# rpacheco-blazquez/PINN-FEM

Measured on AMD Instinct MI355X. Metric: element-residual-grad evals/sec (PINN+GD iteration: MLP fwd+bwd, stiffness, assembly, residual, Adam), collinear truss, higher is better.
Workload: dtype f32; 1 GPU; ex4 shape (nets (20, 15, 10), E and A evaluated), 1000000 elements per GPU, collinear 2-D truss h=1, alpha_data=100 with measurements at every node, load factor 0.1; elements_total=1000000, parallelism=elements sharded x1

## Files before the change

include/pinnfem_hip.h:

```cpp
#ifndef PINNFEM_HIP_H
#define PINNFEM_HIP_H

#include <stdint.h>

#ifdef __cplusplus
extern "C" {
#endif

#define PF_ABI_VERSION 9

#define PF_OK 0
#define PF_ERR_ARG (-1)
#define PF_ERR_UNSUPPORTED (-2)
#define PF_ERR_HIP (-3)

#define PF_DOF_FIXED 1u
#define PF_DOF_MEASURED 2u
#define PF_DOF_SHARED 4u
#define PF_DOF_GHOST 8u

#define PF_WG_SHUFFLE 0
#define PF_WG_MFMA 1
#define PF_WG_MFMA44 2
#define PF_WG_MFMA32 3
// ... 108 lines not shown
int pf_padded_width(int width);
int pf_net_pad_count(int in_dim, int width, int n_hidden);
int pf_net_pad_index(int in_dim, int width, int n_hidden, int local);
int pf_sizeof(int what);
int pf_net_op_count(int in_dim, int width, int n_hidden);
long long pf_partials_count(const pf_problem* p);
#define PF_FUSED_FORWARD 1
#define PF_FUSED_BACKWARD 2
#define PF_FUSED_THETA_UPDATE 4
#define PF_FUSED_U_PINGPONG 8
#define PF_FUSED_U_UPDATE 16
int pf_fusion_info(const pf_problem* p);
#define PF_GRAPH_FORM_FOLDED_RESIDUAL 1
int pf_graph_form_info(const pf_problem* p);
int pf_graph_light_forward(const pf_problem* p);

int pf_pack_theta(const pf_problem* p, void* stream);
int pf_net_forward(const pf_problem* p, int which, void* stream);
int pf_net_forward_all(const pf_problem* p, void* stream);
int pf_net_backward_all(const pf_problem* p, void* stream);
int pf_internal_force(const pf_problem* p, const float* u, float* f_int_out, void* stream);
int pf_node_residual(const pf_problem* p, float* f_int_out, void* stream);
int pf_elem_adjoint(const pf_problem* p, void* stream);
int pf_net_backward(const pf_problem* p, int which, void* stream);
int pf_node_gradu(const pf_problem* p, int fuse_adam, void* stream);
int pf_theta_reduce(const pf_problem* p, int fuse_adam, void* stream);
int pf_finalize(const pf_problem* p, void* stream);
int pf_reset(const pf_problem* p, void* stream);

int pf_gd_iterations(const pf_problem* p, int n_iter, void* stream);
// ... 177 lines not shown
```

pinn_fem_amd/_capi.py:

```python
from __future__ import annotations

import ctypes as C
import os

_HERE = os.path.dirname(os.path.abspath(__file__))
LIB_PATH = os.environ.get("PINNFEM_LIB") or os.path.join(_HERE, "lib", "libpinnfem_hip.so")

PF_ABI_VERSION = 9
PF_OK, PF_ERR_ARG, PF_ERR_UNSUPPORTED, PF_ERR_HIP = 0, -1, -2, -3
PF_DOF_FIXED, PF_DOF_MEASURED, PF_DOF_SHARED, PF_DOF_GHOST = 1, 2, 4, 8
PF_WG_SHUFFLE, PF_WG_MFMA, PF_WG_MFMA44, PF_WG_MFMA32 = 0, 1, 2, 3
PF_N32_WIDTH_MAX = 30
PF_MLP_F32, PF_MLP_BF16 = 0, 1
PF_FE_REFERENCE, PF_FE_DELTA = 0, 1
PF_HIST_COLS = 6
PF_MAX_BLOCKS = 1024
PF_COMM_ID_BYTES = 128
PF_MAX_NODE_BLOCKS = 4096
PF_NODE_SLOTS = PF_MAX_NODE_BLOCKS + 8
PF_KERNEL_SLOTS = 9
PF_COARSE_MAX_AGG, PF_COARSE_MODES = 256, 3
PF_COARSE_MAX = PF_COARSE_MAX_AGG * PF_COARSE_MODES
PF_PCG_MAX_RHS = 2
PF_DYN_ENERGY_COUNT = 4 + 4 * PF_MAX_NODE_BLOCKS
# ... 102 lines not shown
_PD = C.POINTER(PfDyn)
_PH = C.POINTER(PfDynHist)
SYMBOLS = {
    "pf_abi_version": (C.c_int, []),
    "pf_last_error": (C.c_char_p, []),
    "pf_net_param_count": (C.c_int, [C.c_int, C.c_int, C.c_int]),
    "pf_padded_width": (C.c_int, [C.c_int]),
    "pf_net_pad_count": (C.c_int, [C.c_int, C.c_int, C.c_int]),
    "pf_net_pad_index": (C.c_int, [C.c_int, C.c_int, C.c_int, C.c_int]),
    "pf_sizeof": (C.c_int, [C.c_int]),
    "pf_net_op_count": (C.c_int, [C.c_int, C.c_int, C.c_int]),
    "pf_partials_count": (C.c_longlong, [_PP]),
    "pf_fusion_info": (C.c_int, [_PP]),
    "pf_graph_form_info": (C.c_int, [_PP]),
    "pf_graph_light_forward": (C.c_int, [_PP]),
    "pf_pack_theta": (C.c_int, [_PP, C.c_void_p]),
    "pf_net_forward": (C.c_int, [_PP, C.c_int, C.c_void_p]),
    "pf_net_forward_all": (C.c_int, [_PP, C.c_void_p]),
    "pf_net_backward_all": (C.c_int, [_PP, C.c_void_p]),
    "pf_internal_force": (C.c_int, [_PP, C.c_void_p, C.c_void_p, C.c_void_p]),
    "pf_node_residual": (C.c_int, [_PP, C.c_void_p, C.c_void_p]),
    "pf_elem_adjoint": (C.c_int, [_PP, C.c_void_p]),
    "pf_net_backward": (C.c_int, [_PP, C.c_int, C.c_void_p]),
    "pf_node_gradu": (C.c_int, [_PP, C.c_int, C.c_void_p]),
    "pf_theta_reduce": (C.c_int, [_PP, C.c_int, C.c_void_p]),
    "pf_finalize": (C.c_int, [_PP, C.c_void_p]),
    "pf_reset": (C.c_int, [_PP, C.c_void_p]),
    "pf_gd_iterations": (C.c_int, [_PP, C.c_int, C.c_void_p]),
    "pf_graph_create": (C.c_int, [_PP, C.c_int, C.c_void_p, C.POINTER(C.c_void_p)]),
    "pf_graph_create_ex": (C.c_int, [_PP, C.c_int, C.c_int, C.c_void_p, C.POINTER(C.c_void_p)]),
# ... 141 lines not shown
```

pinn_fem_amd/csrc/pf_api.hip:

```cpp
#include <stdlib.h>
#include <string.h>
#include <stdio.h>
#include "pf_common.h"
#include "pf_graph.h"
#include "pf_net32.h"

int pf_launch_node_residual(const pf_problem* p, float* f_int_out, int compute_loss, hipStream_t s, int fin_prev = 0);
int pf_launch_elem_adjoint(const pf_problem* p, hipStream_t s);
int pf_launch_node_gradu(const pf_problem* p, int fuse_adam, hipStream_t s, int skip_shared = 0, float* u_out = nullptr);
int pf_launch_u_home(const pf_problem* p, hipStream_t s);
int pf_launch_scalar_residual(const pf_problem* p, const pf_scalar_id* sp, hipStream_t s);
int pf_launch_scalar_update(const pf_problem* p, const pf_scalar_id* sp, hipStream_t s);
int pf_launch_shard_pack(const pf_problem* p, float* buf2, const float* u2_local, hipStream_t s);
int pf_launch_shard_update(const pf_problem* p, const float* buf2, float* u2_local, hipStream_t s);
int pf_launch_shard_flush(const pf_problem* p, const float* u2, hipStream_t s);
int pf_launch_theta_reduce(const pf_problem* p, int fuse_adam, hipStream_t s);
int pf_launch_pack_theta(const pf_problem* p, hipStream_t s);
int pf_launch_finalize(const pf_problem* p, int mode, int with_theta, hipStream_t s, int tn_ready = 0);
int pf_launch_theta_stage1(const pf_problem* p, hipStream_t s);
int pf_launch_theta_stage1_path(const pf_problem* p, hipStream_t s, int fin_prev);
int pf_launch_path_check(const pf_problem* p, int* bad, hipStream_t s);
int pf_launch_theta_stage2(const pf_problem* p, int fuse_adam, hipStream_t s);
int pf_launch_reset(const pf_problem* p, hipStream_t s);
int pf_launch_adam(float* param, const float* grad, float* m, float* v, int n, int step, double lr,
// ... 440 lines not shown
}

#define PF_CAP_EV 2

static bool pad_index_is_canonical(const pf_problem* p) {
  const int n = p->n_theta_active;
  if (n <= 0 || !p->pad_index) return false;
  int* h = new int[n];
  const bool ok = hipMemcpy(h, p->pad_index, (size_t)n * sizeof(int), hipMemcpyDeviceToHost) == hipSuccess;
  bool same = ok;
  for (int q = 0; same && q < n; ++q) same = h[q] == pf_pad_index_of(*p, q);
  delete[] h;
  return same;
}

static bool mesh_is_path(const pf_problem* p) {
  const pf_mesh& M = p->mesh;
  if (M.n_elems < 1 || M.n_nodes != M.n_elems + 1 || !M.conn || !M.adj_ptr || !M.adj || !M.dof_flags) return false;
  int* bad = nullptr;
  if (hipMalloc(&bad, sizeof(int)) != hipSuccess) {
    pf_set_error("path check of the mesh failed (hipMalloc): the iteration graph keeps its residual launch");
    return false;
  }
  int h = 1;
  bool ok = hipMemset(bad, 0, sizeof(int)) == hipSuccess && pf_launch_path_check(p, bad, nullptr) == PF_OK &&
            hipMemcpy(&h, bad, sizeof(int), hipMemcpyDeviceToHost) == hipSuccess;
  (void)hipFree(bad);
  if (!ok) pf_set_error("path check of the mesh failed (HIP error): the iteration graph keeps its residual launch");
  return ok && h == 0;
}

static bool can_fold_residual_static(const pf_problem* p) {
  return p->prop_double != 0 && p->elem_k != nullptr && p->u_alt != nullptr && can_fuse_gradu(p) && can_fuse_backward(p) &&
         can_fuse_theta_update(p) && pf_n32_bwd2_has_path(p) && p->n_iface == 0 && p->mesh.dim == p->net[0].in_dim - 1;
}
static bool can_fold_residual(const pf_problem* p) { return can_fold_residual_static(p) && mesh_is_path(p); }
static bool can_light_forward(const pf_problem* p, bool fold) {
  return fold && p->net[0].enabled && p->net[1].enabled && pf_n32_has_light_forward(p);
}

static pf_problem graph_iteration_view(const pf_problem& p, int i) {
  pf_problem q = p;
  if (p.prop_double != 0 && (i & 1)) {
    q.prop_e += q.mesh.n_elems;
    q.prop_a += q.mesh.n_elems;
    if (q.elem_k) q.elem_k += (size_t)q.mesh.n_elems * (q.mesh.dim == 2 ? 3 : 1);
  }
  q.part_half = i & 1;
  return q;
}

static int enqueue_graph_iterations(const pf_problem* p, int iters, const pf_capture& c, bool calc_index = false,
                                    bool head_cont = false, bool no_tail = false, bool fold = false) {
  hipStream_t s = c.s;
  if (!(p->net[0].enabled || p->net[1].enabled)) {
    for (int i = 0; i < iters; ++i) {
      int rc = enqueue_iteration(p, 1, 0, s, nullptr);
      if (rc != PF_OK) return rc;
    }
    return PF_OK;
  }
  const bool fuse_gu = p->prop_double != 0 && p->elem_k != nullptr && can_fuse_gradu(p);
  const bool dag = !fuse_gu && p->mesh.n_elems >= PF_GRAPH_DAG_MIN_ELEMS;
  const bool upp = dag && p->u_alt != nullptr && (iters % 2) == 0;
  const bool fuse_s2 = can_fuse_theta_update(p);
  const int tn_ready = p->wg_mode == PF_WG_MFMA32 ? 1 : 0;
  const size_t k_half = (size_t)p->mesh.n_elems * (p->mesh.dim == 2 ? 3 : 1);
  const bool light = can_light_forward(p, fold);
// ... 1 lines not shown
    hipEvent_t* e = c.ev + PF_CAP_EV * i;
    hipEvent_t* ep = c.ev + PF_CAP_EV * (i - 1);
    pf_problem q = graph_iteration_view(*p, i);
    float* u_next = nullptr;
    if (upp) {
      u_next = (i & 1) ? q.u : q.u_alt;
      if (i & 1) q.u = q.u_alt;
    }
    const bool carries = i > 0 || head_cont;
    pf_fwd2_opts fo;
    if (fuse_s2 && carries) fo.s2_half = (i - 1) & 1;
    fo.calc_index = calc_index;
    if (fuse_gu && carries) {
      fo.gu_nb = pf_node_blocks(q.mesh.n_nodes);
      fo.gu_k = p->elem_k + (((i - 1) & 1) ? k_half : 0);
    }
    if (dag && i > 0 && p->prop_double == 0 && hipStreamWaitEvent(s, ep[1], 0) != hipSuccess)
      return fail(PF_ERR_HIP, "graph edge failed");
    fo.light = light ? 1 : 0;
    PF_TRY(net_forward_all(&q, s, fo), "net_forward");
    if (fold) {
      PF_TRY(net_backward2(&q, s, light ? 2 : 1), "net_backward2");
      PF_TRY(pf_launch_theta_stage1_path(&q, s, carries ? (tn_ready ? 2 : 1) : 0), "theta_stage1");
      if (i == iters - 1 && !no_tail) {
        PF_TRY(pf_launch_theta_stage2(&q, 1, s), "theta_stage2");
        PF_TRY(pf_launch_node_gradu(&q, 1, s, 0, nullptr), "node_gradu");
      }
      continue;
    }
    if (dag && i > 0 && hipStreamWaitEvent(s, ep[1], 0) != hipSuccess) return fail(PF_ERR_HIP, "graph edge failed");
// ... 18 lines not shown
  q.part_half = (iters - 1) & 1;
  PF_TRY(pf_launch_finalize(&q, 0, 0, s, tn_ready), "finalize");
  return PF_OK;
}

int pf_graph_form_info(const pf_problem* p) {
  if (check_problem(p) != PF_OK) return PF_ERR_ARG;
  return can_fold_residual(p) ? PF_GRAPH_FORM_FOLDED_RESIDUAL : 0;
}

int pf_graph_light_forward(const pf_problem* p) {
  if (check_problem(p) != PF_OK) return PF_ERR_ARG;
  return can_light_forward(p, can_fold_residual(p)) ? 1 : 0;
}

int pf_graph_create(const pf_problem* p, int iters_per_graph, void* stream, void** graph_out) {
  return pf_graph_create_ex(p, iters_per_graph, 0, stream, graph_out);
}

static bool can_chain_replays(const pf_problem* p, int iters) {
  return (iters % 2) == 0 && p->prop_double != 0 && p->elem_k != nullptr && can_fuse_gradu(p) && can_fuse_theta_update(p);
}

int pf_graph_create_ex(const pf_problem* p, int iters_per_graph, int flags, void* stream, void** graph_out) {
  int rc = check_gd(p);
  if (rc) return rc;
  if (!graph_out || iters_per_graph < 1) return fail(PF_ERR_ARG, "pf_graph_create_ex: bad argument");
  if ((flags & (PF_GRAPH_CONT_HEAD | PF_GRAPH_NO_TAIL)) && !can_chain_replays(p, iters_per_graph))
    return fail(PF_ERR_UNSUPPORTED, "pf_graph_create_ex: replays of this problem's graph cannot hand over their tail");
  const bool calc_index = can_fuse_theta_update(p) && pad_index_is_canonical(p);
  const bool fold = can_fold_residual(p);
  const bool head = (flags & PF_GRAPH_CONT_HEAD) != 0, no_tail = (flags & PF_GRAPH_NO_TAIL) != 0;
  return capture_graph((hipStream_t)stream, PF_CAP_EV * iters_per_graph, hipStreamCaptureModeThreadLocal, graph_out,
                       [&](pf_capture& cap) { return enqueue_graph_iterations(p, iters_per_graph, cap, calc_index, head, no_tail, fold); });
}

int pf_graph_tail(const pf_problem* p, int iters_per_graph, void* stream) {
  int rc = check_gd(p);
  if (rc) return rc;
  if (!can_chain_replays(p, iters_per_graph)) return fail(PF_ERR_UNSUPPORTED, "pf_graph_tail: not a chained replay");
  hipStream_t s = (hipStream_t)stream;
  const pf_problem q = graph_iteration_view(*p, iters_per_graph - 1);
  PF_TRY(pf_launch_theta_stage2(&q, 1, s), "theta_stage2");
  PF_TRY(pf_launch_node_gradu(&q, 1, s, 0, nullptr), "node_gradu");
  PF_TRY(pf_launch_finalize(&q, 0, 0, s, q.wg_mode == PF_WG_MFMA32 ? 1 : 0), "finalize");
  return PF_OK;
}

int pf_graph_launch(void* graph, void* stream) {
// ... 219 lines not shown
```

pinn_fem_amd/csrc/pf_common.h:

```cpp
#pragma once
#include <hip/hip_runtime.h>
#include <stdint.h>
#include <stdlib.h>
#include "pinnfem_hip.h"

#define PF_WAVE 64

#define PF_PART_R2H(h) ((h) ? 3 * PF_NODE_SLOTS : 0)
#define PF_PART_D2H(h) ((h) ? 4 * PF_NODE_SLOTS : PF_NODE_SLOTS)
#define PF_PART_U2 (2 * PF_NODE_SLOTS)
#define PF_PART_WG (5 * PF_NODE_SLOTS)
#define PF_RG 16

#define PF_NET_THREADS 128
#define PF_NODE_THREADS 256

__host__ __device__ constexpr int pf_pad_w1(int) { return 0; }
__host__ __device__ constexpr int pf_pad_wh(int hp, int l ) {
  return hp * 4 + (l - 2) * hp * (hp + 4);
}
__host__ __device__ constexpr int pf_pad_wo(int hp, int nh) {
  return hp * 4 + (nh - 1) * hp * (hp + 4);
}
__host__ __device__ constexpr int pf_pad_count(int hp, int nh) {
// ... 302 lines not shown
PF_DECL_NET_LAUNCHERS(4)
PF_DECL_NET_LAUNCHERS(8)
PF_DECL_NET_LAUNCHERS(12)
PF_DECL_NET_LAUNCHERS(16)
PF_DECL_NET_LAUNCHERS(20)
PF_DECL_NET_LAUNCHERS(24)
PF_DECL_NET_LAUNCHERS(28)
PF_DECL_NET_LAUNCHERS(32)

struct pf_fwd2_opts {
  int s2_half = -1;
  bool calc_index = false;
  int gu_nb = 0;
  const float* gu_k = nullptr;
  int light = 0;
};
#define PF_DECL_NET32_LAUNCHERS(NRB)                                                       \
  int pf_launch_net32_forward_##NRB(const pf_problem* p, int which, hipStream_t s, int s2_half); \
  int pf_launch_net32_backward_##NRB(const pf_problem* p, int which, hipStream_t s);      \
  int pf_launch_net32_backward_gea_##NRB(const pf_problem* p, int which, hipStream_t s);  \
  int pf_launch_net32b_forward_##NRB(const pf_problem* p, int which, hipStream_t s, int s2_half); \
  int pf_launch_net32b_backward_##NRB(const pf_problem* p, int which, hipStream_t s);     \
  int pf_launch_net32b_backward_gea_##NRB(const pf_problem* p, int which, hipStream_t s); \
  int pf_launch_net32_forward2_##NRB(const pf_problem* p, hipStream_t s, const pf_fwd2_opts& o);    \
  int pf_launch_net32b_forward2_##NRB(const pf_problem* p, hipStream_t s, const pf_fwd2_opts& o);   \
  int pf_launch_net32_backward2_##NRB(const pf_problem* p, hipStream_t s, int path);      \
  int pf_launch_net32b_backward2_##NRB(const pf_problem* p, hipStream_t s, int path);
PF_DECL_NET32_LAUNCHERS(2)
PF_DECL_NET32_LAUNCHERS(4)
PF_DECL_NET32_LAUNCHERS(6)
// ... 15 lines not shown
```

pinn_fem_amd/csrc/pf_mesh.hip:

```cpp
#include <stdlib.h>
#include "pf_common.h"
#include "pf_node.h"
#include "pf_net32.h"


namespace {

template <int DIM>
__device__ __forceinline__ void gather_kv(const pf_problem& P, const float* __restrict__ v, int node,
                                          float* acc, bool own_only = false) {
  const pf_mesh& M = P.mesh;
#pragma unroll
  for (int c = 0; c < DIM; ++c) acc[c] = 0.f;
  const int b = M.adj_ptr[node], e_ = M.adj_ptr[node + 1];
  if (P.adj_other) {
    float vs[2];
    load_vec<DIM>(v, node, vs);
    for (int idx = b; idx < e_; idx += 2) {
      const bool two = idx + 1 < e_;
      const int code0 = M.adj[idx], oth0 = P.adj_other[idx];
      const int code1 = two ? M.adj[idx + 1] : code0, oth1 = two ? P.adj_other[idx + 1] : oth0;
      const int e0 = code0 >> 1, e1 = code1 >> 1;
      const ElemK k0 = load_k<DIM>(P, e0), k1 = load_k<DIM>(P, e1);
      float vo0[2], vo1[2], fe[2];
// ... 250 lines not shown
      if (ok[m]) {
#pragma unroll
        for (int c = 0; c < DIM; ++c) dof_loss_terms(fl[m][c], r[m][c], P.use_data, mv[m][c], un[m][c], sum_r2, sum_d2);
      }
  }
  const float t0 = pf_block_sum(sum_r2, red);
  const float t1 = pf_block_sum(sum_d2, red);
  if (threadIdx.x == 0) {
    P.partials[PF_PART_R2H(P.part_half) + bid] = t0;
    P.partials[PF_PART_D2H(P.part_half) + bid] = t1;
  }
}

__global__ __launch_bounds__(256) void k_path_check(pf_mesh M, int* bad) {
  const int n = M.n_elems;
  bool wrong = false;
  for (int e = blockIdx.x * blockDim.x + threadIdx.x; e < n; e += gridDim.x * blockDim.x) {
    const int i = M.conn[2 * e], j = M.conn[2 * e + 1];
    if (i < 0 || i >= M.n_nodes || j < 0 || j >= M.n_nodes) { wrong = true; continue; }
    const int bi = M.adj_ptr[i], di = M.adj_ptr[i + 1] - bi;
    const int bj = M.adj_ptr[j], dj = M.adj_ptr[j + 1] - bj;
    if (e == 0) wrong |= di != 1 || M.adj[bi] != 0;
    else wrong |= di != 2 || M.adj[bi] != (((e - 1) << 1) | 1) || M.adj[bi + 1] != (e << 1);
    if (e == n - 1) wrong |= dj != 1 || M.adj[bj] != ((e << 1) | 1);
    else wrong |= dj != 2 || M.adj[bj] != ((e << 1) | 1) || M.adj[bj + 1] != ((e + 1) << 1);
    for (int c = 0; c < M.dim; ++c)
      wrong |= ((M.dof_flags[i * M.dim + c] | M.dof_flags[j * M.dim + c]) & (PF_DOF_SHARED | PF_DOF_GHOST)) != 0;
  }
  if (wrong) *bad = 1;
}

__device__ __forceinline__ void pack_net_ops(const pf_problem& P, const float* th) {
  if (P.wg_mode != PF_WG_MFMA32 || !P.net_op) return;
  for (int k = 0; k < 2; ++k) {
    if (!P.net[k].enabled) continue;
    pf_n32_pack(P.net[k], th + P.net[k].theta_off, reinterpret_cast<unsigned char*>(P.net_op + P.op_off[k]),
                P.mlp_dtype);
  }
}

__device__ __forceinline__ void theta_update_standalone(const pf_problem& P, int fuse_adam, float* new_theta, int done) {
  const int half = (fuse_adam && P.theta_alt) ? P.state->theta_half : 0;
  if (done) {
    if (half != 0)
// ... 621 lines not shown
```

pinn_fem_amd/csrc/pf_net32.hip:

```cpp
#include <type_traits>
#include <stdlib.h>
#include "pf_net32.h"
#include "pf_node.h"

#ifndef PF_NR
#error "compile with -DPF_NR=<registers per lane>"
#endif
#ifndef PF_PREC
#define PF_PREC 0
#endif
#ifndef PF_N32_DBG_ENABLE
#define PF_N32_DBG_ENABLE 0
#endif
#define PF_CAT2(a, b) a##b
#define PF_CAT(a, b) PF_CAT2(a, b)

typedef _Float16 h2 __attribute__((ext_vector_type(2)));
typedef _Float16 h8 __attribute__((ext_vector_type(8)));
typedef short s4v __attribute__((ext_vector_type(4)));
typedef float f32x16 __attribute__((ext_vector_type(16)));
typedef unsigned u32x4 __attribute__((ext_vector_type(4)));
typedef unsigned u32x2 __attribute__((ext_vector_type(2)));
typedef __bf16 bf2 __attribute__((ext_vector_type(2)));
typedef __bf16 bf8 __attribute__((ext_vector_type(8)));
// ... 778 lines not shown
      out[e] = v;
      if (ws) store_k<IN - 1>(P.elem_k, e, g, (which == 0 ? v * o : o * v) / g.l0);
    }
    if (grp == 3) __builtin_amdgcn_s_barrier();
  }
  if ((dbg & 16) && lane == 0) {
    unsigned long long* d = reinterpret_cast<unsigned long long*>(P.partials) + (size_t)(blockIdx.x * waves + wv) * 4 + (size_t)which * 65536;
    d[0] = sr0; d[1] = __builtin_amdgcn_s_memrealtime(); d[2] = __builtin_amdgcn_s_memtime() - st0;
    unsigned xcc; asm volatile("s_getreg_b32 %0, hwreg(HW_REG_XCC_ID)" : "=s"(xcc));
    unsigned hwid; asm volatile("s_getreg_b32 %0, hwreg(HW_REG_HW_ID)" : "=s"(hwid));
    d[3] = ((unsigned long long)rounds << 48) | ((unsigned long long)(xcc & 0xf) << 32) | hwid;
  }
}

#define PF_GU_MAX_TASKS 1024
template <int NRE, int NRA, int L, int IN, bool LIGHT = false>
__global__ __launch_bounds__(FW_THREADS) void k_net32_forward2(pf_problem P, int dbg_arg, int s2_half, int gu_nb,
                                                               const float* __restrict__ gu_k) {
  using EE = Eng<NRE>;
  using EA = Eng<NRA>;
  const bool calc_index = s2_half >= 2;
  if (calc_index) s2_half -= 2;
  const int dbg = PF_N32_DBG_ENABLE ? dbg_arg : 0;
  extern __shared__ __align__(16) unsigned char smem[];
  constexpr int IMG = pf_n32_bytes(L), IMGP = (IMG + 255) & ~255;
  const unsigned char* __restrict__ img_e = smem;
  const unsigned char* __restrict__ img_a = smem + IMGP;
  const pf_net net_e = P.net[0], net_a = P.net[1];
  if (s2_half < 0) {
    copy_images2(smem, reinterpret_cast<const unsigned char*>(P.net_op + P.op_off[0]), smem + IMGP,
                 reinterpret_cast<const unsigned char*>(P.net_op + P.op_off[1]), IMG);
  }
  const int lane = threadIdx.x & 63, waves = blockDim.x >> 6;
// ... 30 lines not shown
  constexpr int GUN = 64 * PF_GU_M;
  const int n_ntasks = gu_nb > 0 ? (P.mesh.n_nodes + GUN - 1) / GUN : 0;
  const int npb = (n_ntasks + (int)gridDim.x - 1) / (int)gridDim.x;
  const int nt0 = (int)blockIdx.x * npb, nn_b = max(min(nt0 + npb, n_ntasks) - nt0, 0);
  const int gu_every = nn_b > 0 ? max((t1 - t0) / nn_b, 0) : 0;
  bool gu = nn_b > 0;
  int since = nn_b > 0 ? wv % (gu_every + 1) : 0;
  __shared__ int s_done;
  unsigned long long* dstamps = nullptr;
  auto node_task = [&]() {
    int k = 0;
    if (lane == 0) k = atomicAdd(&s_next_n, 1);
    k = __builtin_amdgcn_readfirstlane(k);
    if (k >= nn_b) return false;
    const __attribute__((address_space(4))) pf_problem* pk = kernarg_problem();
    const NodeView NV = node_view_from(pk);
    const GraduConsts GK = gradu_consts_from(pk);
    float su = node_gradu_task<IN - 1, PF_GU_M>(NV, gu_k, GK, (nt0 + k) * GUN, lane);
    su = pf_wave_sum(su);
    if (lane == 0) s_u2[k] = su;
    return true;
  };
  if (s2_half >= 0) {
    if (PF_N32_DBG_ENABLE && (dbg & 16)) {
      dstamps = reinterpret_cast<unsigned long long*>(P.u_alt) + (size_t)(blockIdx.x * waves + wv) * 8;
      if (lane == 0) dstamps[0] = __builtin_amdgcn_s_memrealtime();
    }
    fwd_theta_prologue(P, s2_half, smem, smem + IMGP, reinterpret_cast<float*>(smem + 2 * IMGP), IMG, &s_done, calc_index,
                       (dstamps && lane == 0) ? dstamps : nullptr);
    if (dstamps && lane == 0) dstamps[4] = __builtin_amdgcn_s_memrealtime();
  } else {
    if (threadIdx.x == 0) s_done = P.state->done;
    __syncthreads();
// ... 74 lines not shown
        prop_e[e] = ve;
        prop_a[e] = va;
      }
      if (rec) store_k<IN - 1>(rec, e, g, (ve * va) / g.l0);
    }
    task = nxt;
  }
  if (dstamps && lane == 0) dstamps[5] = __builtin_amdgcn_s_memrealtime();
  if (gu_nb > 0) {
    __syncthreads();
    float su = 0.f;
    for (int i = threadIdx.x; i < nn_b; i += blockDim.x) su += s_u2[i];
    float* red = reinterpret_cast<float*>(s_u2 + PF_GU_MAX_TASKS - 16);
    __syncthreads();
    su = pf_block_sum(su, red);
    if (threadIdx.x == 0) P.partials[PF_PART_U2 + blockIdx.x] = su;
    for (int j = (int)blockIdx.x + (int)gridDim.x + (int)threadIdx.x * (int)gridDim.x; j < gu_nb; j += (int)blockDim.x * (int)gridDim.x)
      P.partials[PF_PART_U2 + j] = 0.f;
  }
}

template <int L>
constexpr int bw_park_floats() { return L * 1024 + 64; }
template <int NR, int L>
__device__ __forceinline__ void bw_park(float* __restrict__ mine, const f32x16 (&T)[L], const float (&go)[NR], float gbo, int lane) {
  const int h = lane >> 5;
  sfor<0, L>([&](auto l) {
    constexpr int LL = l;
    sfor<0, 16>([&](auto i) {
      constexpr int I = i;
      const int m = (I & 3) + 8 * (I >> 2) + 4 * h;
      mine[LL * 1024 + m * 32 + (lane & 31)] = T[LL][I];
    });
// ... 471 lines not shown

template <int NRA, int L, int IN>
int launch_fwd2_t(const pf_problem* p, hipStream_t s, const pf_fwd2_opts& o) {
  const int s2_half = o.s2_half, gu_nb = o.gu_nb;
  constexpr int NRE = PF_NR;
  const int n = p->mesh.n_elems;
  const int nb = pf_n32_fwd2_blocks(n);
  static const int dbg = getenv("PF_N32_DBG") ? atoi(getenv("PF_N32_DBG")) : 0;
  const size_t lds = 2 * (size_t)((pf_n32_bytes(L) + 255) & ~255) + (s2_half < 0 ? 0 : (size_t)p->n_theta_active * sizeof(float));
  if (lds > 64000) { pf_set_error("too many trainable parameters for the fused theta update"); return PF_ERR_UNSUPPORTED; }
  if (gu_nb > 0 && !pf_n32_fwd2_can_update_u(p, gu_nb)) { pf_set_error("fused forward: displacement update not possible on this problem"); return PF_ERR_UNSUPPORTED; }
  const int s2_arg = s2_half >= 0 && o.calc_index ? s2_half + 2 : s2_half;
  if (o.light) {
    if constexpr (n32_has_light<NRE, NRA, L, IN>()) {
      if (!p->elem_k) { pf_set_error("fused forward, light form: elem_k is needed"); return PF_ERR_ARG; }
      hipLaunchKernelGGL((k_net32_forward2<NRE, NRA, L, IN, true>), dim3(nb), dim3(FW_THREADS), lds, s, *p, dbg, s2_arg, gu_nb, o.gu_k);
    } else {
      pf_set_error("fused forward: no light form for these nets");
      return PF_ERR_UNSUPPORTED;
    }
  } else {
    hipLaunchKernelGGL((k_net32_forward2<NRE, NRA, L, IN>), dim3(nb), dim3(FW_THREADS), lds, s, *p, dbg, s2_arg, gu_nb, o.gu_k);
  }
  return hipGetLastError() == hipSuccess ? PF_OK : PF_ERR_HIP;
}
template <int L, int IN>
int launch_fwd2(const pf_problem* p, hipStream_t s, const pf_fwd2_opts& o) {
  switch (pf_net32_bucket(p->net[1].width)) {
    case 2: return launch_fwd2_t<2, L, IN>(p, s, o);
    case 4: return launch_fwd2_t<4, L, IN>(p, s, o);
    case 6: return launch_fwd2_t<6, L, IN>(p, s, o);
    case 8: return launch_fwd2_t<8, L, IN>(p, s, o);
    case 10: return launch_fwd2_t<10, L, IN>(p, s, o);
    case 12: return launch_fwd2_t<12, L, IN>(p, s, o);
    case 15: return launch_fwd2_t<15, L, IN>(p, s, o);
  }
  pf_set_error("MFMA32 engine: area net width outside 1..30");
// ... 122 lines not shown
```

pinn_fem_amd/csrc/pf_node.h:

```cpp
#pragma once
#include "pf_common.h"

struct GraduConsts { float step_size, bc2s, b1w, b2, b2w, eps, dcoef; };

template <class PP>
__device__ __forceinline__ GraduConsts gradu_consts_from(PP p) {
  GraduConsts K;
  const pf_state* st = p->state;
  K.step_size = st->step_size_u;
  K.bc2s = st->bc2_sqrt;
  K.b1w = (float)(1.0 - p->beta1);
  K.b2 = (float)p->beta2;
  K.b2w = (float)(1.0 - p->beta2);
  K.eps = (float)p->eps;
  const float nm = p->n_meas_f;
  K.dcoef = nm > 0.f ? p->alpha_data / nm : 0.f;
  return K;
}
__device__ __forceinline__ GraduConsts gradu_consts(const pf_problem& P) { return gradu_consts_from(&P); }

struct NodeView {
  const int32_t *adj_ptr, *adj, *adj_other;
  const uint8_t* dof_flags;
  const float *meas_val, *g_f;
  float *u, *m_u, *v_u, *grad_u;
  int n_nodes, use_data, fe_mode;
};
template <class PP>
__device__ __forceinline__ NodeView node_view_from(PP p) {
  NodeView V;
  V.adj_ptr = p->mesh.adj_ptr;
  V.adj = p->mesh.adj;
  V.adj_other = p->adj_other;
  V.dof_flags = p->mesh.dof_flags;
  V.meas_val = p->mesh.meas_val;
  V.g_f = p->g_f;
  V.u = p->u;
  V.m_u = p->m_u;
  V.v_u = p->v_u;
  V.grad_u = p->grad_u;
  V.n_nodes = p->mesh.n_nodes;
  V.use_data = p->use_data;
  V.fe_mode = p->fe_mode;
  return V;
}

__device__ __forceinline__ float dof_grad_u(const GraduConsts& K, bool measured, float g, float meas, float uo) {
  PF_NO_CONTRACT
// ... 3 lines not shown
    gu += -(K.dcoef * (2.f * d));
  }
  return gu;
}

__device__ __forceinline__ void dof_adam_u(const GraduConsts& K, float gu, float& uo, float& m, float& v) {
  PF_NO_CONTRACT
  m = m + K.b1w * (gu - m);
  v = v * K.b2;
  v = v + (K.b2w * gu) * gu;
  const float denom = sqrtf(v) / K.bc2s + K.eps;
  uo = uo + (-K.step_size) * (m / denom);
}

template <int DIM, int M>
__device__ __forceinline__ float node_gradu_task(const NodeView& P, const float* __restrict__ elem_k, const GraduConsts& K,
                                                 int node0, int lane) {
  const int nn = P.n_nodes;
  int node[M], b[M], e_[M];
  bool ok[M];
  float vs[M][2], acc[M][2], uo[M][2], meas[M][2];
  unsigned fl[M][2];
  const float* __restrict__ mvals = P.use_data ? P.meas_val : P.u;
#pragma unroll
  for (int m = 0; m < M; ++m) {
    const int n_ = node0 + m * 64 + lane;
    ok[m] = n_ < nn;
    node[m] = ok[m] ? n_ : nn - 1;
    b[m] = P.adj_ptr[node[m]];
    e_[m] = P.adj_ptr[node[m] + 1];
    load_vec<DIM>(P.g_f, node[m], vs[m]);
    load_vec<DIM>(P.u, node[m], uo[m]);
#pragma unroll
    for (int c = 0; c < DIM; ++c) {
      fl[m][c] = P.dof_flags[node[m] * DIM + c];
      meas[m][c] = mvals[node[m] * DIM + c];
      acc[m][c] = 0.f;
    }
  }
  int rounds = 0;
#pragma unroll
  for (int m = 0; m < M; ++m) rounds = max(rounds, (e_[m] - b[m] + 1) >> 1);
  float mo[M][2], vo[M][2];
#pragma unroll
  for (int m = 0; m < M; ++m)
#pragma unroll
    for (int c = 0; c < DIM; ++c) {
      mo[m][c] = P.m_u[node[m] * DIM + c];
      vo[m][c] = P.v_u[node[m] * DIM + c];
    }
  for (int r = 0; r < rounds; ++r) {
    int code0[M], code1[M], oth0[M], oth1[M];
    bool has[M], two[M];
#pragma unroll
    for (int m = 0; m < M; ++m) {
      const int idx = b[m] + 2 * r;
      has[m] = idx < e_[m];
      two[m] = idx + 1 < e_[m];
      const int i0 = has[m] ? idx : 0, i1 = two[m] ? idx + 1 : i0;
      code0[m] = P.adj[i0];
      oth0[m] = P.adj_other[i0];
      code1[m] = P.adj[i1];
      oth1[m] = P.adj_other[i1];
    }
    ElemK k0[M], k1[M];
    float w0[M][2], w1[M][2];
#pragma unroll
    for (int m = 0; m < M; ++m) {
      k0[m] = load_k_record<DIM>(elem_k, code0[m] >> 1);
      k1[m] = load_k_record<DIM>(elem_k, code1[m] >> 1);
      load_vec<DIM>(P.g_f, oth0[m], w0[m]);
      load_vec<DIM>(P.g_f, oth1[m], w1[m]);
    }
#pragma unroll
    for (int m = 0; m < M; ++m) {
      float fe[2];
      const int end0 = code0[m] & 1, end1 = code1[m] & 1;
      ke_rows_times<DIM>(k0[m], end0, end0 ? w0[m] : vs[m], end0 ? vs[m] : w0[m], fe, P.fe_mode);
#pragma unroll
      for (int c = 0; c < DIM; ++c) {
        const float t = acc[m][c] + fe[c];
        acc[m][c] = has[m] ? t : acc[m][c];
      }
      ke_rows_times<DIM>(k1[m], end1, end1 ? w1[m] : vs[m], end1 ? vs[m] : w1[m], fe, P.fe_mode);
#pragma unroll
      for (int c = 0; c < DIM; ++c) {
        const float t = acc[m][c] + fe[c];
        acc[m][c] = two[m] ? t : acc[m][c];
      }
    }
#pragma unroll
    for (int m = 0; m < M; ++m)
#pragma unroll
      for (int c = 0; c < DIM; ++c)
        asm volatile("" : "+v"(uo[m][c]), "+v"(meas[m][c]), "+v"(mo[m][c]), "+v"(vo[m][c]));
  }
  float sum_u2 = 0.f;
#pragma unroll
  for (int m = 0; m < M; ++m) {
#pragma unroll
    for (int c = 0; c < DIM; ++c) {
      const int dof = node[m] * DIM + c;
      const unsigned f = fl[m][c];
      const float gu = dof_grad_u(K, P.use_data && (f & PF_DOF_MEASURED), acc[m][c], meas[m][c], uo[m][c]);
      float un = uo[m][c], mn = mo[m][c], vn = vo[m][c];
      dof_adam_u(K, gu, un, mn, vn);
      const bool fixed = (f & PF_DOF_FIXED) != 0;
      if (ok[m]) {
        if (P.grad_u) P.grad_u[dof] = gu;
        if (fixed) {
          if (uo[m][c] != 0.f) P.u[dof] = 0.f;
        } else {
          P.m_u[dof] = mn;
          P.v_u[dof] = vn;
          P.u[dof] = un;
        }
      }
      { PF_NO_CONTRACT
        if (ok[m] && !fixed) sum_u2 += un * un; }
    }
  }
  return sum_u2;
}

template <int DIM, int M>
__device__ __forceinline__ void gather_kv_multi(const pf_problem& P, const float* __restrict__ elem_k,
                                                const float* __restrict__ v, const int (&node)[M], float (&acc)[M][2]) {
  const pf_mesh& Ms = P.mesh;
  int b[M], e_[M];
  float vs[M][2];
#pragma unroll
  for (int m = 0; m < M; ++m) {
    b[m] = Ms.adj_ptr[node[m]];
    e_[m] = Ms.adj_ptr[node[m] + 1];
    load_vec<DIM>(v, node[m], vs[m]);
    acc[m][0] = 0.f;
    acc[m][1] = 0.f;
  }
  int rounds = 0;
#pragma unroll
// ... 112 lines not shown
```

pinn_fem_amd/engine.py:

```python
from __future__ import annotations

import contextlib
import ctypes as C
import functools
import os
import time
import warnings
from typing import List, Optional

import numpy as np
import torch

from . import _capi
from . import coarse as _coarse
from ._capi import PfProblem, PfState, PinnFemHipError
from .nets import FlatTheta, NetSpec, describe_module
from .plan import HostPlan, build_host_plan


def _require_gpu(device=None) -> torch.device:
    if not torch.cuda.is_available():
        raise PinnFemHipError(
            "no ROCm GPU visible: pinn_fem_amd runs its hot path only through the HIP kernels "
            "(gfx950) and has no CPU fallback")
# ... 278 lines not shown
        view.mesh.dof_flags = flags_t.data_ptr()
        return C.byref(view), mask, key

    def fusion_info(self) -> int:
        return int(self.lib.pf_fusion_info(self._ref()))

    @_on_engine_stream
    def graph_form_info(self) -> int:
        return int(self.lib.pf_graph_form_info(self._ref()))

    @_on_engine_stream
    def graph_light_forward(self) -> int:
        return int(self.lib.pf_graph_light_forward(self._ref()))

    @_on_engine_stream
    def begin(self, u_initial, lam, config, max_iter: Optional[int] = None, want_history=True):
        if self.n_theta and not self.theta.still_bound():
            raise PinnFemHipError("a network parameter was re-assigned outside the engine; "
                                  "rebuild the engine for this model")
        self.configure(lam=lam, alpha_physics=config.alpha_physics, alpha_data=config.alpha_data,
                       lr_u=config.learning_rate_u, lr_t=config.learning_rate_theta,
                       tol=config.tolerance,
                       max_iter=config.max_iterations if max_iter is None else max_iter,
                       want_history=want_history)
        if u_initial is None:
            self.u.zero_()
        else:
            src = u_initial.detach() if isinstance(u_initial, torch.Tensor) else torch.as_tensor(
                np.asarray(u_initial))
            self.u.copy_(src.reshape(-1).to(device=self.device, dtype=torch.float32))
# ... 755 lines not shown
```

Baseline: 8.631 billion element-evals/s.

## Use direct neighbor indexing in fused grad-u when path mesh is ordered

Extends the path check to detect meshes whose elements are numbered sequentially (element e joins nodes e and e+1). When the check passes, the fused forward kernel's grad-u tasks read the stiffness records and neighbor vectors of elements node-1 and node directly, skipping the CSR adjacency lookups (adj_ptr, adj, adj_other) and the round loop. This removes dependent indirect loads on the node update path. It adds a kernel argument, a second code path and a host-side query.

```diff
diff --git a/include/pinnfem_hip.h b/include/pinnfem_hip.h
--- a/include/pinnfem_hip.h
+++ b/include/pinnfem_hip.h
@@ -146,6 +146,7 @@
 #define PF_GRAPH_FORM_FOLDED_RESIDUAL 1
 int pf_graph_form_info(const pf_problem* p);
 int pf_graph_light_forward(const pf_problem* p);
+int pf_graph_ordered_path(const pf_problem* p);
 
 int pf_pack_theta(const pf_problem* p, void* stream);
 int pf_net_forward(const pf_problem* p, int which, void* stream);
diff --git a/pinn_fem_amd/_capi.py b/pinn_fem_amd/_capi.py
--- a/pinn_fem_amd/_capi.py
+++ b/pinn_fem_amd/_capi.py
@@ -140,6 +140,7 @@
     "pf_fusion_info": (C.c_int, [_PP]),
     "pf_graph_form_info": (C.c_int, [_PP]),
     "pf_graph_light_forward": (C.c_int, [_PP]),
+    "pf_graph_ordered_path": (C.c_int, [_PP]),
     "pf_pack_theta": (C.c_int, [_PP, C.c_void_p]),
     "pf_net_forward": (C.c_int, [_PP, C.c_int, C.c_void_p]),
     "pf_net_forward_all": (C.c_int, [_PP, C.c_void_p]),
diff --git a/pinn_fem_amd/csrc/pf_api.hip b/pinn_fem_amd/csrc/pf_api.hip
--- a/pinn_fem_amd/csrc/pf_api.hip
+++ b/pinn_fem_amd/csrc/pf_api.hip
@@ -478,7 +478,8 @@
   return same;
 }
 
-static bool mesh_is_path(const pf_problem* p) {
+static bool mesh_is_path(const pf_problem* p, bool* ordered = nullptr) {
+  if (ordered) *ordered = false;
   const pf_mesh& M = p->mesh;
   if (M.n_elems < 1 || M.n_nodes != M.n_elems + 1 || !M.conn || !M.adj_ptr || !M.adj || !M.dof_flags) return false;
   int* bad = nullptr;
@@ -491,14 +492,18 @@
             hipMemcpy(&h, bad, sizeof(int), hipMemcpyDeviceToHost) == hipSuccess;
   (void)hipFree(bad);
   if (!ok) pf_set_error("path check of the mesh failed (HIP error): the iteration graph keeps its residual launch");
-  return ok && h == 0;
+  if (ordered) *ordered = ok && h == 0;
+  return ok && (h & 1) == 0;
 }
 
 static bool can_fold_residual_static(const pf_problem* p) {
   return p->prop_double != 0 && p->elem_k != nullptr && p->u_alt != nullptr && can_fuse_gradu(p) && can_fuse_backward(p) &&
          can_fuse_theta_update(p) && pf_n32_bwd2_has_path(p) && p->n_iface == 0 && p->mesh.dim == p->net[0].in_dim - 1;
 }
-static bool can_fold_residual(const pf_problem* p) { return can_fold_residual_static(p) && mesh_is_path(p); }
+static bool can_fold_residual(const pf_problem* p, bool* ordered = nullptr) {
+  if (ordered) *ordered = false;
+  return can_fold_residual_static(p) && mesh_is_path(p, ordered);
+}
 static bool can_light_forward(const pf_problem* p, bool fold) {
   return fold && p->net[0].enabled && p->net[1].enabled && pf_n32_has_light_forward(p);
 }
@@ -515,7 +520,7 @@
 }
 
 static int enqueue_graph_iterations(const pf_problem* p, int iters, const pf_capture& c, bool calc_index = false,
-                                    bool head_cont = false, bool no_tail = false, bool fold = false) {
+                                    bool head_cont = false, bool no_tail = false, bool fold = false, bool ordered = false) {
   hipStream_t s = c.s;
   if (!(p->net[0].enabled || p->net[1].enabled)) {
     for (int i = 0; i < iters; ++i) {
@@ -547,6 +552,7 @@
     if (fuse_gu && carries) {
       fo.gu_nb = pf_node_blocks(q.mesh.n_nodes);
       fo.gu_k = p->elem_k + (((i - 1) & 1) ? k_half : 0);
+      fo.gu_ordered = fold && ordered ? 1 : 0;
     }
     if (dag && i > 0 && p->prop_double == 0 && hipStreamWaitEvent(s, ep[1], 0) != hipSuccess)
       return fail(PF_ERR_HIP, "graph edge failed");
@@ -595,6 +601,12 @@
   return can_light_forward(p, can_fold_residual(p)) ? 1 : 0;
 }
 
+int pf_graph_ordered_path(const pf_problem* p) {
+  if (check_problem(p) != PF_OK) return PF_ERR_ARG;
+  bool ordered = false;
+  return can_fold_residual(p, &ordered) && ordered ? 1 : 0;
+}
+
 int pf_graph_create(const pf_problem* p, int iters_per_graph, void* stream, void** graph_out) {
   return pf_graph_create_ex(p, iters_per_graph, 0, stream, graph_out);
 }
@@ -610,10 +622,11 @@
   if ((flags & (PF_GRAPH_CONT_HEAD | PF_GRAPH_NO_TAIL)) && !can_chain_replays(p, iters_per_graph))
     return fail(PF_ERR_UNSUPPORTED, "pf_graph_create_ex: replays of this problem's graph cannot hand over their tail");
   const bool calc_index = can_fuse_theta_update(p) && pad_index_is_canonical(p);
-  const bool fold = can_fold_residual(p);
+  bool ordered = false;
+  const bool fold = can_fold_residual(p, &ordered);
   const bool head = (flags & PF_GRAPH_CONT_HEAD) != 0, no_tail = (flags & PF_GRAPH_NO_TAIL) != 0;
   return capture_graph((hipStream_t)stream, PF_CAP_EV * iters_per_graph, hipStreamCaptureModeThreadLocal, graph_out,
-                       [&](pf_capture& cap) { return enqueue_graph_iterations(p, iters_per_graph, cap, calc_index, head, no_tail, fold); });
+                       [&](pf_capture& cap) { return enqueue_graph_iterations(p, iters_per_graph, cap, calc_index, head, no_tail, fold, ordered); });
 }
 
 int pf_graph_tail(const pf_problem* p, int iters_per_graph, void* stream) {
diff --git a/pinn_fem_amd/csrc/pf_common.h b/pinn_fem_amd/csrc/pf_common.h
--- a/pinn_fem_amd/csrc/pf_common.h
+++ b/pinn_fem_amd/csrc/pf_common.h
@@ -340,6 +340,7 @@
   int gu_nb = 0;
   const float* gu_k = nullptr;
   int light = 0;
+  int gu_ordered = 0;
 };
 #define PF_DECL_NET32_LAUNCHERS(NRB)                                                       \
   int pf_launch_net32_forward_##NRB(const pf_problem* p, int which, hipStream_t s, int s2_half); \
diff --git a/pinn_fem_amd/csrc/pf_mesh.hip b/pinn_fem_amd/csrc/pf_mesh.hip
--- a/pinn_fem_amd/csrc/pf_mesh.hip
+++ b/pinn_fem_amd/csrc/pf_mesh.hip
@@ -288,9 +288,10 @@
 
 __global__ __launch_bounds__(256) void k_path_check(pf_mesh M, int* bad) {
   const int n = M.n_elems;
-  bool wrong = false;
+  bool wrong = false, unordered = false;
   for (int e = blockIdx.x * blockDim.x + threadIdx.x; e < n; e += gridDim.x * blockDim.x) {
     const int i = M.conn[2 * e], j = M.conn[2 * e + 1];
+    unordered |= i != e || j != e + 1;
     if (i < 0 || i >= M.n_nodes || j < 0 || j >= M.n_nodes) { wrong = true; continue; }
     const int bi = M.adj_ptr[i], di = M.adj_ptr[i + 1] - bi;
     const int bj = M.adj_ptr[j], dj = M.adj_ptr[j + 1] - bj;
@@ -301,7 +302,8 @@
     for (int c = 0; c < M.dim; ++c)
       wrong |= ((M.dof_flags[i * M.dim + c] | M.dof_flags[j * M.dim + c]) & (PF_DOF_SHARED | PF_DOF_GHOST)) != 0;
   }
-  if (wrong) *bad = 1;
+  const int bits = (wrong ? 1 : 0) | (unordered ? 2 : 0);
+  if (bits) atomicOr(bad, bits);
 }
 
 __device__ __forceinline__ void pack_net_ops(const pf_problem& P, const float* th) {
diff --git a/pinn_fem_amd/csrc/pf_net32.hip b/pinn_fem_amd/csrc/pf_net32.hip
--- a/pinn_fem_amd/csrc/pf_net32.hip
+++ b/pinn_fem_amd/csrc/pf_net32.hip
@@ -816,9 +816,15 @@
 }
 
 #define PF_GU_MAX_TASKS 1024
+struct fwd2_kernargs {
+  pf_problem P;
+  int dbg_arg, s2_half, gu_nb;
+  const float* gu_k;
+  int gu_ordered;
+};
 template <int NRE, int NRA, int L, int IN, bool LIGHT = false>
 __global__ __launch_bounds__(FW_THREADS) void k_net32_forward2(pf_problem P, int dbg_arg, int s2_half, int gu_nb,
-                                                               const float* __restrict__ gu_k) {
+                                                               const float* __restrict__ gu_k, int gu_ordered) {
   using EE = Eng<NRE>;
   using EA = Eng<NRA>;
   const bool calc_index = s2_half >= 2;
@@ -879,9 +885,18 @@
     k = __builtin_amdgcn_readfirstlane(k);
     if (k >= nn_b) return false;
     const __attribute__((address_space(4))) pf_problem* pk = kernarg_problem();
-    const NodeView NV = node_view_from(pk);
     const GraduConsts GK = gradu_consts_from(pk);
-    float su = node_gradu_task<IN - 1, PF_GU_M>(NV, gu_k, GK, (nt0 + k) * GUN, lane);
+    float su;
+    bool ordered = false;
+    if constexpr (EE::COMPACT && EA::COMPACT)
+      ordered = reinterpret_cast<const __attribute__((address_space(4))) fwd2_kernargs*>(pk)->gu_ordered != 0;
+    if (ordered) {
+      const NodeView NV = node_view_from<false>(pk);
+      su = node_gradu_task_path<IN - 1, PF_GU_M>(NV, gu_k, GK, (nt0 + k) * GUN, lane);
+    } else {
+      const NodeView NV = node_view_from(pk);
+      su = node_gradu_task<IN - 1, PF_GU_M>(NV, gu_k, GK, (nt0 + k) * GUN, lane);
+    }
     su = pf_wave_sum(su);
     if (lane == 0) s_u2[k] = su;
     return true;
@@ -986,9 +1001,13 @@
     float* red = reinterpret_cast<float*>(s_u2 + PF_GU_MAX_TASKS - 16);
     __syncthreads();
     su = pf_block_sum(su, red);
-    if (threadIdx.x == 0) P.partials[PF_PART_U2 + blockIdx.x] = su;
-    for (int j = (int)blockIdx.x + (int)gridDim.x + (int)threadIdx.x * (int)gridDim.x; j < gu_nb; j += (int)blockDim.x * (int)gridDim.x)
-      P.partials[PF_PART_U2 + j] = 0.f;
+    const __attribute__((address_space(4))) fwd2_kernargs* ke =
+        reinterpret_cast<const __attribute__((address_space(4))) fwd2_kernargs*>(kernarg_problem());
+    float* __restrict__ const partials = ke->P.partials;
+    const int n_u2 = ke->gu_nb;
+    if (threadIdx.x == 0) partials[PF_PART_U2 + blockIdx.x] = su;
+    for (int j = (int)blockIdx.x + (int)gridDim.x + (int)threadIdx.x * (int)gridDim.x; j < n_u2; j += (int)blockDim.x * (int)gridDim.x)
+      partials[PF_PART_U2 + j] = 0.f;
   }
 }
 
@@ -1490,13 +1509,13 @@
   if (o.light) {
     if constexpr (n32_has_light<NRE, NRA, L, IN>()) {
       if (!p->elem_k) { pf_set_error("fused forward, light form: elem_k is needed"); return PF_ERR_ARG; }
-      hipLaunchKernelGGL((k_net32_forward2<NRE, NRA, L, IN, true>), dim3(nb), dim3(FW_THREADS), lds, s, *p, dbg, s2_arg, gu_nb, o.gu_k);
+      hipLaunchKernelGGL((k_net32_forward2<NRE, NRA, L, IN, true>), dim3(nb), dim3(FW_THREADS), lds, s, *p, dbg, s2_arg, gu_nb, o.gu_k, o.gu_ordered);
     } else {
       pf_set_error("fused forward: no light form for these nets");
       return PF_ERR_UNSUPPORTED;
     }
   } else {
-    hipLaunchKernelGGL((k_net32_forward2<NRE, NRA, L, IN>), dim3(nb), dim3(FW_THREADS), lds, s, *p, dbg, s2_arg, gu_nb, o.gu_k);
+    hipLaunchKernelGGL((k_net32_forward2<NRE, NRA, L, IN>), dim3(nb), dim3(FW_THREADS), lds, s, *p, dbg, s2_arg, gu_nb, o.gu_k, o.gu_ordered);
   }
   return hipGetLastError() == hipSuccess ? PF_OK : PF_ERR_HIP;
 }
diff --git a/pinn_fem_amd/csrc/pf_node.h b/pinn_fem_amd/csrc/pf_node.h
--- a/pinn_fem_amd/csrc/pf_node.h
+++ b/pinn_fem_amd/csrc/pf_node.h
@@ -26,12 +26,12 @@
   float *u, *m_u, *v_u, *grad_u;
   int n_nodes, use_data, fe_mode;
 };
-template <class PP>
+template <bool ADJ = true, class PP>
 __device__ __forceinline__ NodeView node_view_from(PP p) {
   NodeView V;
-  V.adj_ptr = p->mesh.adj_ptr;
-  V.adj = p->mesh.adj;
-  V.adj_other = p->adj_other;
+  V.adj_ptr = ADJ ? p->mesh.adj_ptr : nullptr;
+  V.adj = ADJ ? p->mesh.adj : nullptr;
+  V.adj_other = ADJ ? p->adj_other : nullptr;
   V.dof_flags = p->mesh.dof_flags;
   V.meas_val = p->mesh.meas_val;
   V.g_f = p->g_f;
@@ -65,87 +65,10 @@
 }
 
 template <int DIM, int M>
-__device__ __forceinline__ float node_gradu_task(const NodeView& P, const float* __restrict__ elem_k, const GraduConsts& K,
-                                                 int node0, int lane) {
-  const int nn = P.n_nodes;
-  int node[M], b[M], e_[M];
-  bool ok[M];
-  float vs[M][2], acc[M][2], uo[M][2], meas[M][2];
-  unsigned fl[M][2];
-  const float* __restrict__ mvals = P.use_data ? P.meas_val : P.u;
-#pragma unroll
-  for (int m = 0; m < M; ++m) {
-    const int n_ = node0 + m * 64 + lane;
-    ok[m] = n_ < nn;
-    node[m] = ok[m] ? n_ : nn - 1;
-    b[m] = P.adj_ptr[node[m]];
-    e_[m] = P.adj_ptr[node[m] + 1];
-    load_vec<DIM>(P.g_f, node[m], vs[m]);
-    load_vec<DIM>(P.u, node[m], uo[m]);
-#pragma unroll
-    for (int c = 0; c < DIM; ++c) {
-      fl[m][c] = P.dof_flags[node[m] * DIM + c];
-      meas[m][c] = mvals[node[m] * DIM + c];
-      acc[m][c] = 0.f;
-    }
-  }
-  int rounds = 0;
-#pragma unroll
-  for (int m = 0; m < M; ++m) rounds = max(rounds, (e_[m] - b[m] + 1) >> 1);
-  float mo[M][2], vo[M][2];
-#pragma unroll
-  for (int m = 0; m < M; ++m)
-#pragma unroll
-    for (int c = 0; c < DIM; ++c) {
-      mo[m][c] = P.m_u[node[m] * DIM + c];
-      vo[m][c] = P.v_u[node[m] * DIM + c];
-    }
-  for (int r = 0; r < rounds; ++r) {
-    int code0[M], code1[M], oth0[M], oth1[M];
-    bool has[M], two[M];
-#pragma unroll
-    for (int m = 0; m < M; ++m) {
-      const int idx = b[m] + 2 * r;
-      has[m] = idx < e_[m];
-      two[m] = idx + 1 < e_[m];
-      const int i0 = has[m] ? idx : 0, i1 = two[m] ? idx + 1 : i0;
-      code0[m] = P.adj[i0];
-      oth0[m] = P.adj_other[i0];
-      code1[m] = P.adj[i1];
-      oth1[m] = P.adj_other[i1];
-    }
-    ElemK k0[M], k1[M];
-    float w0[M][2], w1[M][2];
-#pragma unroll
-    for (int m = 0; m < M; ++m) {
-      k0[m] = load_k_record<DIM>(elem_k, code0[m] >> 1);
-      k1[m] = load_k_record<DIM>(elem_k, code1[m] >> 1);
-      load_vec<DIM>(P.g_f, oth0[m], w0[m]);
-      load_vec<DIM>(P.g_f, oth1[m], w1[m]);
-    }
-#pragma unroll
-    for (int m = 0; m < M; ++m) {
-      float fe[2];
-      const int end0 = code0[m] & 1, end1 = code1[m] & 1;
-      ke_rows_times<DIM>(k0[m], end0, end0 ? w0[m] : vs[m], end0 ? vs[m] : w0[m], fe, P.fe_mode);
-#pragma unroll
-      for (int c = 0; c < DIM; ++c) {
-        const float t = acc[m][c] + fe[c];
-        acc[m][c] = has[m] ? t : acc[m][c];
-      }
-      ke_rows_times<DIM>(k1[m], end1, end1 ? w1[m] : vs[m], end1 ? vs[m] : w1[m], fe, P.fe_mode);
-#pragma unroll
-      for (int c = 0; c < DIM; ++c) {
-        const float t = acc[m][c] + fe[c];
-        acc[m][c] = two[m] ? t : acc[m][c];
-      }
-    }
-#pragma unroll
-    for (int m = 0; m < M; ++m)
-#pragma unroll
-      for (int c = 0; c < DIM; ++c)
-        asm volatile("" : "+v"(uo[m][c]), "+v"(meas[m][c]), "+v"(mo[m][c]), "+v"(vo[m][c]));
-  }
+__device__ __forceinline__ float node_task_update(const NodeView& P, const GraduConsts& K, const int (&node)[M],
+                                                  const bool (&ok)[M], const unsigned (&fl)[M][2], const float (&acc)[M][2],
+                                                  const float (&meas)[M][2], const float (&uo)[M][2],
+                                                  const float (&mo)[M][2], const float (&vo)[M][2]) {
   float sum_u2 = 0.f;
 #pragma unroll
   for (int m = 0; m < M; ++m) {
@@ -175,6 +98,142 @@
 }
 
 template <int DIM, int M>
+__device__ __forceinline__ float node_gradu_task(const NodeView& P, const float* __restrict__ elem_k, const GraduConsts& K,
+                                                 int node0, int lane) {
+  const int nn = P.n_nodes;
+  int node[M], b[M], e_[M];
+  bool ok[M];
+  float vs[M][2], acc[M][2], uo[M][2], meas[M][2];
+  unsigned fl[M][2];
+  const float* __restrict__ mvals = P.use_data ? P.meas_val : P.u;
+#pragma unroll
+  for (int m = 0; m < M; ++m) {
+    const int n_ = node0 + m * 64 + lane;
+    ok[m] = n_ < nn;
+    node[m] = ok[m] ? n_ : nn - 1;
+    b[m] = P.adj_ptr[node[m]];
+    e_[m] = P.adj_ptr[node[m] + 1];
+    load_vec<DIM>(P.g_f, node[m], vs[m]);
+    load_vec<DIM>(P.u, node[m], uo[m]);
+#pragma unroll
+    for (int c = 0; c < DIM; ++c) {
+      fl[m][c] = P.dof_flags[node[m] * DIM + c];
+      meas[m][c] = mvals[node[m] * DIM + c];
+      acc[m][c] = 0.f;
+    }
+  }
+  int rounds = 0;
+#pragma unroll
+  for (int m = 0; m < M; ++m) rounds = max(rounds, (e_[m] - b[m] + 1) >> 1);
+  float mo[M][2], vo[M][2];
+#pragma unroll
+  for (int m = 0; m < M; ++m)
+#pragma unroll
+    for (int c = 0; c < DIM; ++c) {
+      mo[m][c] = P.m_u[node[m] * DIM + c];
+      vo[m][c] = P.v_u[node[m] * DIM + c];
+    }
+  for (int r = 0; r < rounds; ++r) {
+    int code0[M], code1[M], oth0[M], oth1[M];
+    bool has[M], two[M];
+#pragma unroll
+    for (int m = 0; m < M; ++m) {
+      const int idx = b[m] + 2 * r;
+      has[m] = idx < e_[m];
+      two[m] = idx + 1 < e_[m];
+      const int i0 = has[m] ? idx : 0, i1 = two[m] ? idx + 1 : i0;
+      code0[m] = P.adj[i0];
+      oth0[m] = P.adj_other[i0];
+      code1[m] = P.adj[i1];
+      oth1[m] = P.adj_other[i1];
+    }
+    ElemK k0[M], k1[M];
+    float w0[M][2], w1[M][2];
+#pragma unroll
+    for (int m = 0; m < M; ++m) {
+      k0[m] = load_k_record<DIM>(elem_k, code0[m] >> 1);
+      k1[m] = load_k_record<DIM>(elem_k, code1[m] >> 1);
+      load_vec<DIM>(P.g_f, oth0[m], w0[m]);
+      load_vec<DIM>(P.g_f, oth1[m], w1[m]);
+    }
+#pragma unroll
+    for (int m = 0; m < M; ++m) {
+      float fe[2];
+      const int end0 = code0[m] & 1, end1 = code1[m] & 1;
+      ke_rows_times<DIM>(k0[m], end0, end0 ? w0[m] : vs[m], end0 ? vs[m] : w0[m], fe, P.fe_mode);
+#pragma unroll
+      for (int c = 0; c < DIM; ++c) {
+        const float t = acc[m][c] + fe[c];
+        acc[m][c] = has[m] ? t : acc[m][c];
+      }
+      ke_rows_times<DIM>(k1[m], end1, end1 ? w1[m] : vs[m], end1 ? vs[m] : w1[m], fe, P.fe_mode);
+#pragma unroll
+      for (int c = 0; c < DIM; ++c) {
+        const float t = acc[m][c] + fe[c];
+        acc[m][c] = two[m] ? t : acc[m][c];
+      }
+    }
+#pragma unroll
+    for (int m = 0; m < M; ++m)
+#pragma unroll
+      for (int c = 0; c < DIM; ++c)
+        asm volatile("" : "+v"(uo[m][c]), "+v"(meas[m][c]), "+v"(mo[m][c]), "+v"(vo[m][c]));
+  }
+  return node_task_update<DIM, M>(P, K, node, ok, fl, acc, meas, uo, mo, vo);
+}
+
+template <int DIM, int M>
+__device__ __forceinline__ float node_gradu_task_path(const NodeView& P, const float* __restrict__ elem_k,
+                                                      const GraduConsts& K, int node0, int lane) {
+  const int nn = P.n_nodes, ne = nn - 1;
+  int node[M];
+  bool ok[M];
+  float vs[M][2], wb[M][2], wa[M][2], acc[M][2], uo[M][2], meas[M][2], mo[M][2], vo[M][2];
+  unsigned fl[M][2];
+  ElemK kb[M], ka[M];
+  const float* __restrict__ mvals = P.use_data ? P.meas_val : P.u;
+#pragma unroll
+  for (int m = 0; m < M; ++m) {
+    const int n_ = node0 + m * 64 + lane;
+    ok[m] = n_ < nn;
+    node[m] = ok[m] ? n_ : nn - 1;
+    const int below = max(node[m] - 1, 0), above = min(node[m] + 1, nn - 1);
+    kb[m] = load_k_record<DIM>(elem_k, below);
+    ka[m] = load_k_record<DIM>(elem_k, min(node[m], ne - 1));
+    load_vec<DIM>(P.g_f, below, wb[m]);
+    load_vec<DIM>(P.g_f, node[m], vs[m]);
+    load_vec<DIM>(P.g_f, above, wa[m]);
+    load_vec<DIM>(P.u, node[m], uo[m]);
+#pragma unroll
+    for (int c = 0; c < DIM; ++c) {
+      fl[m][c] = P.dof_flags[node[m] * DIM + c];
+      meas[m][c] = mvals[node[m] * DIM + c];
+      mo[m][c] = P.m_u[node[m] * DIM + c];
+      vo[m][c] = P.v_u[node[m] * DIM + c];
+      acc[m][c] = 0.f;
+    }
+  }
+#pragma unroll
+  for (int m = 0; m < M; ++m) {
+    const bool has_b = node[m] > 0, has_a = node[m] < ne;
+    float fe[2];
+    ke_rows_times<DIM>(kb[m], 1, wb[m], vs[m], fe, P.fe_mode);
+#pragma unroll
+    for (int c = 0; c < DIM; ++c) {
+      const float t = acc[m][c] + fe[c];
+      acc[m][c] = has_b ? t : acc[m][c];
+    }
+    ke_rows_times<DIM>(ka[m], 0, vs[m], wa[m], fe, P.fe_mode);
+#pragma unroll
+    for (int c = 0; c < DIM; ++c) {
+      const float t = acc[m][c] + fe[c];
+      acc[m][c] = has_a ? t : acc[m][c];
+    }
+  }
+  return node_task_update<DIM, M>(P, K, node, ok, fl, acc, meas, uo, mo, vo);
+}
+
+template <int DIM, int M>
 __device__ __forceinline__ void gather_kv_multi(const pf_problem& P, const float* __restrict__ elem_k,
                                                 const float* __restrict__ v, const int (&node)[M], float (&acc)[M][2]) {
   const pf_mesh& Ms = P.mesh;
diff --git a/pinn_fem_amd/engine.py b/pinn_fem_amd/engine.py
--- a/pinn_fem_amd/engine.py
+++ b/pinn_fem_amd/engine.py
@@ -316,6 +316,10 @@
         return int(self.lib.pf_graph_light_forward(self._ref()))
 
     @_on_engine_stream
+    def graph_ordered_path(self) -> int:
+        return int(self.lib.pf_graph_ordered_path(self._ref()))
+
+    @_on_engine_stream
     def begin(self, u_initial, lam, config, max_iter: Optional[int] = None, want_history=True):
         if self.n_theta and not self.theta.still_bound():
             raise PinnFemHipError("a network parameter was re-assigned outside the engine; "
```

Measured after the change: 8.920 billion element-evals/s, median of 6. 3.4% higher.
